# AndrewRLawrence/dp_gp_lvm

Hardware: AMD Instinct MI355X
Metric: ELBO evals/sec (N=2000,D=512,M=128,Q=10) (higher is better)
Workload: dtype f32 (psi-statistics: f16 hi/lo-split MFMA operands, fp32 accumulate) + f64 (Cholesky chain)

## Files before the change

### dp_gp_lvm_amd/csrc/psi2_pairs.hip

```cpp
#include <type_traits>
#include "internal.h"
#include "psi2_consts.h"
#include "psi2_chain_task.h"

typedef _Float16 pp_h8 __attribute__((ext_vector_type(8)));
typedef _Float16 pp_h2 __attribute__((ext_vector_type(2)));
typedef float pp_f16v __attribute__((ext_vector_type(16)));

#define PP_APAD 8
#define PP_LDS_HDR 512

#ifndef PP_G
#define PP_G(KS) ((KS) <= 4 ? 6 : ((KS) <= 6 ? 4 : 2))
#endif
#ifndef PP_WAVES
#define PP_WAVES 2
#endif
template <int KS> struct PairsCfg { static constexpr int G = PP_G(KS); };

#ifndef PP_NW8_MIN_TILES
#define PP_NW8_MIN_TILES 512
#endif
#ifndef PP_DEEP_PREFETCH
#define PP_DEEP_PREFETCH 1
#endif
#ifndef PP_SCALAR_ADD
#define PP_SCALAR_ADD 1
#endif

template <int KS, int GG, int NW>
__device__ __forceinline__ void pairs_load(pp_h8 (&bop)[GG][KS], int tb, const _Float16 *__restrict__ img, int l5, int half) {
#pragma unroll
    for (int g = 0; g < GG; ++g) {
        const pp_h8 *row = reinterpret_cast<const pp_h8 *>(img) + (size_t)(tb + NW * g) * KS * 64 + 32 * half + l5;
#pragma unroll
        for (int ks = 0; ks < KS; ++ks) bop[g][ks] = row[ks * 64];
    }
}

template <int KS, int GG, int NW>
__device__ __forceinline__ void pairs_group(int tb, pp_h8 (&bop)[GG][KS], int tb_next, const _Float16 *__restrict__ aimg,
                                            const _Float16 *__restrict__ img,
                                            const unsigned *__restrict__ pmap, const float *__restrict__ scale, int ntile,
                                            int l5, int half, float poison, float *__restrict__ out, int Mp, int chunk) {
    constexpr int SLP = 16 * KS, LDA = SLP + PP_APAD;
    static_assert(GG == 1 || (GG & 1) == 0, "ping-pong needs an even number of resident tiles");
    unsigned pm[GG];
    float sc[GG], old[GG];
#pragma unroll
    for (int g = 0; g < GG; ++g) {
        pm[g] = pmap[32 * (tb + NW * g) + l5];
        sc[g] = scale[32 * (tb + NW * g) + l5];
    }
#pragma unroll
    for (int g = 0; g < GG; ++g) {
        old[g] = 0.0f;
        if (chunk && pm[g] != 0xffffffffu && half == 0) old[g] = out[(size_t)(pm[g] >> 16) * Mp + (pm[g] & 0xffffu)];
    }
    float acc[GG][4];
#pragma unroll
    for (int g = 0; g < GG; ++g)
#pragma unroll
        for (int i = 0; i < 4; ++i) acc[g][i] = 0.0f;
    const _Float16 *arow = aimg + (size_t)l5 * LDA + 8 * half;
    auto load_a = [&](pp_h8 (&a)[KS], int nt) __attribute__((always_inline)) {
#ifdef PP_DIAG_NO_ALOAD
        if (nt > 1) return;
#endif
#pragma unroll
        for (int ks = 0; ks < KS; ++ks) a[ks] = *reinterpret_cast<const pp_h8 *>(arow + (size_t)nt * 32 * LDA + 16 * ks);
    };
    auto mma = [&](pp_f16v &c, const pp_h8 (&a)[KS], const pp_h8 (&bq)[KS]) __attribute__((always_inline)) {
#pragma unroll
        for (int v = 0; v < 16; ++v) c[v] = 0.0f;
#pragma unroll
        for (int ks = 0; ks < KS; ++ks) c = __builtin_amdgcn_mfma_f32_32x32x16_f16(a[ks], bq[ks], c, 0, 0, 0);
    };
    auto stage = [&](pp_f16v &cn, const pp_h8 (&a)[KS], const pp_h8 (&bq)[KS], float (&ac)[4], const pp_f16v &cu)
                     __attribute__((always_inline)) {
#pragma unroll
        for (int v = 0; v < 16; ++v) cn[v] = 0.0f;
#ifndef PP_MFMA_PER_STEP
#define PP_MFMA_PER_STEP 1
#endif
#pragma unroll
        for (int ks = 0; ks < KS; ks += PP_MFMA_PER_STEP) {
#ifndef PP_DIAG_NO_MFMA
#pragma unroll
            for (int k2 = ks; k2 < ks + PP_MFMA_PER_STEP && k2 < KS; ++k2)
                cn = __builtin_amdgcn_mfma_f32_32x32x16_f16(a[k2], bq[k2], cn, 0, 0, 0);
#endif
            __builtin_amdgcn_sched_barrier(0);
            const int kend = (ks + PP_MFMA_PER_STEP < KS) ? ks + PP_MFMA_PER_STEP : KS;
            const int v0 = (16 * ks) / KS, v1 = (16 * kend) / KS;
#pragma unroll
            for (int v = v0; v < v1; ++v) {
#ifdef PP_DIAG_NO_EXP
                const float e = cu[v];
#else
                const float e = __builtin_amdgcn_exp2f(cu[v]);
#endif
#if PP_SCALAR_ADD
                asm("v_add_f32 %0, %0, %1" : "+v"(ac[v & 3]) : "v"(e));
#else
                ac[v & 3] += e;
#endif
            }
            __builtin_amdgcn_sched_barrier(0);
        }
    };
    pp_f16v c0, c1;
    if constexpr (GG == 2 && PP_DEEP_PREFETCH) {
        pp_h8 a0[KS], a1[KS], a2[KS];
        load_a(a0, 0);
        load_a(a1, min(1, ntile - 1));
        mma(c0, a0, bop[0]);
#pragma unroll 1
        for (int nt = 0; nt < ntile; nt += 3) {
            load_a(a2, min(nt + 2, ntile - 1));
            stage(c1, a0, bop[1], acc[0], c0);
            stage(c0, a1, bop[0], acc[1], c1);
            if (nt + 1 >= ntile) break;
            load_a(a0, min(nt + 3, ntile - 1));
            stage(c1, a1, bop[1], acc[0], c0);
            stage(c0, a2, bop[0], acc[1], c1);
            if (nt + 2 >= ntile) break;
            load_a(a1, min(nt + 4, ntile - 1));
            stage(c1, a2, bop[1], acc[0], c0);
            stage(c0, a0, bop[0], acc[1], c1);
        }
    } else {
        pp_h8 a_0[KS], a_1[KS];
        load_a(a_0, 0);
        mma(c0, a_0, bop[0]);
        auto row = [&](const pp_h8 (&a_cur)[KS], const pp_h8 (&a_nxt)[KS]) __attribute__((always_inline)) {
            if constexpr (GG == 1) {
                stage(c1, a_nxt, bop[0], acc[0], c0);
                c0 = c1;
            } else {
#pragma unroll
                for (int g = 0; g < GG; g += 2) {
                    stage(c1, a_cur, bop[g + 1], acc[g], c0);
                    if (g + 2 < GG) stage(c0, a_cur, bop[g + 2], acc[g + 1], c1);
                    else stage(c0, a_nxt, bop[0], acc[g + 1], c1);
                }
            }
        };
#pragma unroll 1
        for (int nt = 0; nt < ntile; nt += 2) {
            load_a(a_1, min(nt + 1, ntile - 1));
            row(a_0, a_1);
            if (nt + 1 >= ntile) break;
            load_a(a_0, min(nt + 2, ntile - 1));
            row(a_1, a_0);
        }
    }
    if (tb_next >= 0) pairs_load<KS, GG, NW>(bop, tb_next, img, l5, half);
#pragma unroll
    for (int g = 0; g < GG; ++g) {
        float tot = (acc[g][0] + acc[g][1]) + (acc[g][2] + acc[g][3]);
        tot += __shfl_xor(tot, 32, 64);
        if (pm[g] != 0xffffffffu && half == 0)
            out[(size_t)(pm[g] >> 16) * Mp + (pm[g] & 0xffffu)] = old[g] + (sc[g] * tot + poison);
    }
}

template <typename TIN>
__global__ __launch_bounds__(256) void psi2_pair_scale_kernel(int M, int Q, const TIN *__restrict__ z,
                                                              const TIN *__restrict__ gamma, const TIN *__restrict__ alpha,
                                                              float *__restrict__ scale) {
    psi2_pair_scale_block<TIN, TIN>((int)blockIdx.y, (int)blockIdx.x, M, Q, z, gamma, alpha, scale);
}

template <typename TIN, int KS, int NW>
__global__ __launch_bounds__(64 * NW, PP_WAVES) void psi2_pairs_kernel(int N, int M, int Q, int B, const unsigned char *__restrict__ consts,
                                                            const TIN *__restrict__ mu, const TIN *__restrict__ s,
                                                            const TIN *__restrict__ gamma, const float *__restrict__ scale,
                                                            float *__restrict__ part, int Mp, int n_per_split, int n_splits,
                                                            int n_ranges, int tiles_per_range, int R, ChainKTask task) {
    constexpr int G = PairsCfg<KS>::G, SLP = 16 * KS, LDA = SLP + PP_APAD;
    extern __shared__ __align__(16) unsigned char smem_raw[];
    int item;
    if (psi2_task_1d(blockIdx.x, task.ws ? B : 0, task.last != 0, item)) {
#ifndef PP_NO_CHAIN
        if constexpr (std::is_same<TIN, double>::value && NW == 4) chain_k_task<2>(task, item, smem_raw);
#endif
        return;
    }
    const int b = item % B, sp = (item / B) % n_splits, rg = item / (B * n_splits);
    float *gq = reinterpret_cast<float *>(smem_raw);
    float *zc = gq + 32;
    _Float16 *aimg = reinterpret_cast<_Float16 *>(smem_raw + PP_LDS_HDR);
    const Psi2Consts C = psi2_consts_layout(M, Q);
    const _Float16 *img = reinterpret_cast<const _Float16 *>(consts + C.off_pairs);
    const unsigned *pmap = reinterpret_cast<const unsigned *>(consts + C.off_pmap);
    const float *sc_b = scale + (size_t)b * C.Ppad;
    const int t = threadIdx.x, lane = t & 63, l5 = lane & 31, half = lane >> 5;
    const int wv = __builtin_amdgcn_readfirstlane(t >> 6);
    if (t < 32) {
        gq[t] = (t < Q) ? (float)gamma[(size_t)b * Q + t] : 0.0f;
        zc[t] = reinterpret_cast<const float *>(consts)[t];
    }
    const int tiles_total = C.Ppad / 32;
    const int t0 = rg * tiles_per_range, t1 = min(tiles_total, t0 + tiles_per_range);
    const int nbeg = sp * n_per_split, nend = min(N, nbeg + n_per_split);
    float poison = 0.0f;
    float *out = part + ((size_t)sp * B + b) * (size_t)Mp * Mp;
    bool oor = false;
    __syncthreads();

    for (int n0 = nbeg, chunk = 0; n0 < nend; n0 += R, ++chunk) {
        const int rows = min(R, nend - n0), ntile = (rows + 31) >> 5;
        if (chunk) __syncthreads();
        for (int r = t; r < 32 * ntile; r += 64 * NW) {
            const int n = n0 + r;
            unsigned *dst = reinterpret_cast<unsigned *>(aimg + (size_t)r * LDA);
            float cc = -60000.0f;
            if (n < nend) {
                cc = 0.0f;
                for (int q = 0; q < Q; ++q) {
                    const float g = gq[q], sv = (float)s[(size_t)n * Q + q], mc = (float)mu[(size_t)n * Q + q] - zc[q];
                    const float den = 2.0f * g * sv + 1.0f, w = g / den;
                    const float a = dpgp_pin((float)(-0.25 * DPGP_LOG2E / PSI2_PAIR_S2_SCALE) * w);
                    const float bb = dpgp_pin((float)DPGP_LOG2E * w * mc);
                    cc -= bb * mc + 0.5f * __builtin_amdgcn_logf(den);
                    const _Float16 ah = (_Float16)a, alo = (_Float16)(a - (float)ah);
                    const _Float16 bh = (_Float16)bb, blo = (_Float16)(bb - (float)bh);
                    const pp_h2 w0 = {ah, ah}, w1 = {alo, bh}, w2 = {bh, blo};
                    dst[3 * q] = __builtin_bit_cast(unsigned, w0);
                    dst[3 * q + 1] = __builtin_bit_cast(unsigned, w1);
                    dst[3 * q + 2] = __builtin_bit_cast(unsigned, w2);
                }
                oor |= !(cc >= -8192.0f);
                cc = fmaxf(cc, -60000.0f);
            } else {
                for (int q = 0; q < 3 * Q; ++q) dst[q] = 0u;
            }
            cc = dpgp_pin(cc);
            const _Float16 ch = (_Float16)cc;
            const float r1 = dpgp_pin(cc - (float)ch);
            const _Float16 cm = (_Float16)r1;
            const pp_h2 cw = {ch, cm}, cw2 = {(_Float16)(r1 - (float)cm), (_Float16)0.0f};
            dst[3 * Q] = __builtin_bit_cast(unsigned, cw);
            for (int k = 3 * Q + 1; k < SLP / 2; ++k) dst[k] = 0u;
            if (6 * Q + 2 < SLP) dst[3 * Q + 1] = __builtin_bit_cast(unsigned, cw2);
        }
        if (__syncthreads_or(oor ? 1 : 0)) poison = __builtin_nanf("");

        int tb = t0 + wv;
        if (tb + NW * (G - 1) < t1) {
            pp_h8 bop[G][KS];
            pairs_load<KS, G, NW>(bop, tb, img, l5, half);
            for (; tb + NW * (G - 1) < t1; tb += NW * G) {
                const int nx = tb + NW * G;
                pairs_group<KS, G, NW>(tb, bop, nx + NW * (G - 1) < t1 ? nx : -1, aimg, img, pmap, sc_b, ntile, l5, half, poison, out,
                                   Mp, chunk);
            }
        }
        if constexpr (G > 2)
            for (; tb + NW < t1; tb += 2 * NW) {
                pp_h8 bop[2][KS];
                pairs_load<KS, 2, NW>(bop, tb, img, l5, half);
                pairs_group<KS, 2, NW>(tb, bop, -1, aimg, img, pmap, sc_b, ntile, l5, half, poison, out, Mp, chunk);
            }
        for (; tb < t1; tb += NW) {
            pp_h8 bop[1][KS];
            pairs_load<KS, 1, NW>(bop, tb, img, l5, half);
            pairs_group<KS, 1, NW>(tb, bop, -1, aimg, img, pmap, sc_b, ntile, l5, half, poison, out, Mp, chunk);
        }
    }
}

struct PairsGeom {
    int KS, R, n_ranges, tiles_per_range, NW;
    size_t lds;
};
static PairsGeom pairs_geom(int B, int N, int M, int Q, int ns, size_t chain_lds) {
    const Psi2Consts C = psi2_consts_layout(M, Q);
    PairsGeom g;
    g.KS = C.KS;
    const size_t row = sizeof(_Float16) * (size_t)(16 * C.KS + PP_APAD);
    size_t budget = 80 * 1024;
    if (const char *e = getenv("DPGP_PP_LDS_KB")) budget = (size_t)atoi(e) * 1024;
    if (chain_lds > budget) budget = chain_lds;
    int rmax = (int)((budget - PP_LDS_HDR) / row) & ~31;
    const int nper = dpgp_ceil_div(N, ns);
    g.NW = (!chain_lds && nper > rmax && C.Ppad / 32 >= PP_NW8_MIN_TILES) ? 8 : 4;
    if (const char *e = getenv("DPGP_PP_NW")) {
        const int v = atoi(e);
        if ((v == 4 || v == 8) && !(v == 8 && chain_lds)) g.NW = v;
    }
    if (g.NW == 8) {
        budget = 160 * 1024;
        rmax = (int)((budget - PP_LDS_HDR) / row) & ~31;
    }
    int r = dpgp_round_up(nper, 32);
    if (r > rmax) {
        const int chunks = dpgp_ceil_div(nper, rmax);
        r = dpgp_round_up(dpgp_ceil_div(nper, chunks), 32);
    }
    g.R = r;
    g.lds = PP_LDS_HDR + row * (size_t)r;
    if (chain_lds > g.lds) g.lds = chain_lds;
    const int tiles = C.Ppad / 32;
    int nr = chain_lds ? (B < 128 ? 512 - B : 512) / (B * ns) : dpgp_ceil_div(g.NW == 8 ? 256 : 512, B * ns);
    if (nr > dpgp_ceil_div(tiles, 32)) nr = dpgp_ceil_div(tiles, 32);
    if (nr < 1) nr = 1;
    if (const char *e = getenv("DPGP_PP_RANGES")) {
        const int v = atoi(e);
        if (v >= 1 && v <= tiles) nr = v;
    }
    g.tiles_per_range = dpgp_ceil_div(tiles, nr);
    g.n_ranges = dpgp_ceil_div(tiles, g.tiles_per_range);
    return g;
}

template <typename TIN, int KS, int NW>
static int launch_pairs_ks(int B, int N, int M, int Q, const TIN *mu, const TIN *s, const TIN *gamma, const float *scale,
                           float *part, int ns, const ChainKTask &task, const unsigned char *consts, const PairsGeom &g,
                           hipStream_t st) {
    const int Mp = dpgp_round_up(M, 16);
    const int nper = dpgp_ceil_div(N, ns);
    const long long nwg = (long long)B * ns * g.n_ranges + (task.ws ? B : 0);
    if (nwg > 0x7fffffffLL) return -1;
    auto kern = psi2_pairs_kernel<TIN, KS, NW>;
    if (NW == 8 && task.ws) return -16;
    if (g.lds > 48 * 1024 &&
        hipFuncSetAttribute(reinterpret_cast<const void *>(kern), hipFuncAttributeMaxDynamicSharedMemorySize, (int)g.lds) !=
            hipSuccess)
        return DPGP_ERR_LAUNCH;
    DPGP_PRELAUNCH(); hipLaunchKernelGGL(kern, dim3((unsigned)nwg), dim3(64 * NW), g.lds, st, N, M, Q, B, consts, mu, s, gamma, scale, part,
                       Mp, nper, ns, g.n_ranges, g.tiles_per_range, g.R, task);
    DPGP_LAUNCH_CHECK();
    return DPGP_OK;
}

size_t psi2_pairs_scale_bytes(int B, int M) {
    const size_t ppad = ((size_t)M * (M + 1) / 2 + 31) & ~(size_t)31;
    return dpgp_align256(sizeof(float) * (size_t)B * ppad);
}
template <typename TIN>
int launch_psi2_pairs(int B, int N, int M, int Q, const TIN *z, const TIN *mu, const TIN *s, const TIN *gamma,
                      const TIN *alpha, float *part, int ns, const ChainKTask &task, const unsigned char *consts, float *scale,
                      int scale_ready, hipStream_t st) {
    if (!consts || !scale) return -18;
    if (!scale_ready) {
        const Psi2Consts C = psi2_consts_layout(M, Q);
        DPGP_PRELAUNCH(); hipLaunchKernelGGL((psi2_pair_scale_kernel<TIN>), dim3(dpgp_ceil_div(C.Ppad, 256), B), dim3(256), 0, st, M, Q, z,
                           gamma, alpha, scale);
        DPGP_LAUNCH_CHECK();
    }
    size_t chain_lds = 0;
    if (task.ws) {
        if (!chain_k_resident(task.Mp, task.elem)) return -16;
        chain_lds = chain_k_lds_bytes(task.Mp, task.elem);
    }
    const PairsGeom g = pairs_geom(B, N, M, Q, ns, chain_lds);
    switch (g.KS) {
#define CASE(k)                                                                                                       \
    case k:                                                                                                           \
        return g.NW == 8 ? launch_pairs_ks<TIN, k, 8>(B, N, M, Q, mu, s, gamma, scale, part, ns, task, consts, g, st) \
                         : launch_pairs_ks<TIN, k, 4>(B, N, M, Q, mu, s, gamma, scale, part, ns, task, consts, g, st);
        CASE(2) CASE(4) CASE(6) CASE(8)
#undef CASE
    }
    return -4;
}
template int launch_psi2_pairs<float>(int, int, int, int, const float *, const float *, const float *, const float *,
                                      const float *, float *, int, const ChainKTask &, const unsigned char *, float *, int,
                                      hipStream_t);
template int launch_psi2_pairs<double>(int, int, int, int, const double *, const double *, const double *, const double *,
                                       const double *, float *, int, const ChainKTask &, const unsigned char *, float *, int,
                                       hipStream_t);
```

Before: 778.5.

## Stage mu/s rows through LDS with coalesced loads and defer old-output reads

Before building the A image, mu and s for the chunk are loaded cooperatively with coalesced, unrolled global reads and written into the tail of each LDS row. The per-row encode loop then reads them from LDS instead of making strided per-thread global loads. In the pair groups, the read of the previous partial output is moved after the MFMA loop, and explicit waitcnt calls let the MFMA loop wait only on the B-operand loads rather than on every outstanding memory op. This reuses LDS row padding as scratch and depends on hand-coded waitcnt encodings, which risks ordering bugs if the load counts assumed in those encodings are off.

New measurement: 785.5, median of 6. No clear change (+0.9%).

```diff
diff --git a/dp_gp_lvm_amd/csrc/psi2_pairs.hip b/dp_gp_lvm_amd/csrc/psi2_pairs.hip
--- a/dp_gp_lvm_amd/csrc/psi2_pairs.hip
+++ b/dp_gp_lvm_amd/csrc/psi2_pairs.hip
@@ -26,6 +26,10 @@
 #endif
 #ifndef PP_SCALAR_ADD
 #define PP_SCALAR_ADD 1
+#endif
+
+#ifndef PP_STAGE_U
+#define PP_STAGE_U 8
 #endif
 
 template <int KS, int GG, int NW>
@@ -46,16 +50,11 @@
     constexpr int SLP = 16 * KS, LDA = SLP + PP_APAD;
     static_assert(GG == 1 || (GG & 1) == 0, "ping-pong needs an even number of resident tiles");
     unsigned pm[GG];
-    float sc[GG], old[GG];
+    float sc[GG];
 #pragma unroll
     for (int g = 0; g < GG; ++g) {
         pm[g] = pmap[32 * (tb + NW * g) + l5];
         sc[g] = scale[32 * (tb + NW * g) + l5];
-    }
-#pragma unroll
-    for (int g = 0; g < GG; ++g) {
-        old[g] = 0.0f;
-        if (chunk && pm[g] != 0xffffffffu && half == 0) old[g] = out[(size_t)(pm[g] >> 16) * Mp + (pm[g] & 0xffffu)];
     }
     float acc[GG][4];
 #pragma unroll
@@ -109,12 +108,14 @@
             __builtin_amdgcn_sched_barrier(0);
         }
     };
+    auto bop_wait = [&]() __attribute__((always_inline)) { __builtin_amdgcn_s_waitcnt(0x0f70 | (2 * GG)); };
     pp_f16v c0, c1;
     if constexpr (GG == 2 && PP_DEEP_PREFETCH) {
         pp_h8 a0[KS], a1[KS], a2[KS];
         load_a(a0, 0);
         load_a(a1, min(1, ntile - 1));
         mma(c0, a0, bop[0]);
+        bop_wait();
 #pragma unroll 1
         for (int nt = 0; nt < ntile; nt += 3) {
             load_a(a2, min(nt + 2, ntile - 1));
@@ -133,6 +134,7 @@
         pp_h8 a_0[KS], a_1[KS];
         load_a(a_0, 0);
         mma(c0, a_0, bop[0]);
+        bop_wait();
         auto row = [&](const pp_h8 (&a_cur)[KS], const pp_h8 (&a_nxt)[KS]) __attribute__((always_inline)) {
             if constexpr (GG == 1) {
                 stage(c1, a_nxt, bop[0], acc[0], c0);
@@ -155,14 +157,25 @@
             row(a_1, a_0);
         }
     }
+    unsigned off[GG];
+    float old[GG];
+#pragma unroll
+    for (int g = 0; g < GG; ++g) {
+        off[g] = (pm[g] != 0xffffffffu && half == 0) ? (pm[g] >> 16) * (unsigned)Mp + (pm[g] & 0xffffu) : 0xffffffffu;
+        old[g] = 0.0f;
+        if (chunk && off[g] != 0xffffffffu) old[g] = out[off[g]];
+    }
     if (tb_next >= 0) pairs_load<KS, GG, NW>(bop, tb_next, img, l5, half);
+    float tot[GG];
 #pragma unroll
     for (int g = 0; g < GG; ++g) {
-        float tot = (acc[g][0] + acc[g][1]) + (acc[g][2] + acc[g][3]);
-        tot += __shfl_xor(tot, 32, 64);
-        if (pm[g] != 0xffffffffu && half == 0)
-            out[(size_t)(pm[g] >> 16) * Mp + (pm[g] & 0xffffu)] = old[g] + (sc[g] * tot + poison);
-    }
+        tot[g] = (acc[g][0] + acc[g][1]) + (acc[g][2] + acc[g][3]);
+        tot[g] += __shfl_xor(tot[g], 32, 64);
+    }
+    __builtin_amdgcn_s_waitcnt(0x0f70);
+#pragma unroll
+    for (int g = 0; g < GG; ++g)
+        if (off[g] != 0xffffffffu) out[off[g]] = old[g] + (sc[g] * tot[g] + poison);
 }
 
 template <typename TIN>
@@ -212,14 +225,48 @@
     for (int n0 = nbeg, chunk = 0; n0 < nend; n0 += R, ++chunk) {
         const int rows = min(R, nend - n0), ntile = (rows + 31) >> 5;
         if (chunk) __syncthreads();
+        const int SW = LDA / 2 - 2 * Q;
+        {
+            const int ne = rows * Q;
+            const TIN *mu0 = mu + (size_t)n0 * Q, *s0 = s + (size_t)n0 * Q;
+            int tq = t;
+            asm volatile("" : "+v"(tq));
+            const int er_d = __builtin_amdgcn_readfirstlane((64 * NW) / Q), eq_d = 64 * NW - er_d * Q;
+            int er = tq / Q, eq = tq - er * Q;
+            for (int e0 = t; e0 < ne; e0 += PP_STAGE_U * 64 * NW) {
+                TIN mv[PP_STAGE_U], sv[PP_STAGE_U];
+#pragma unroll
+                for (int u = 0; u < PP_STAGE_U; ++u) {
+                    const int e = min(e0 + u * 64 * NW, ne - 1);
+                    mv[u] = mu0[e];
+                    sv[u] = s0[e];
+                }
+#pragma unroll
+                for (int u = 0; u < PP_STAGE_U; ++u) {
+                    if (e0 + u * 64 * NW < ne) {
+                        float2 *slot = reinterpret_cast<float2 *>(reinterpret_cast<float *>(aimg + (size_t)er * LDA) + SW) + eq;
+                        *slot = make_float2((float)mv[u], (float)sv[u]);
+                    }
+                    er += er_d;
+                    eq += eq_d;
+                    if (eq >= Q) {
+                        eq -= Q;
+                        ++er;
+                    }
+                }
+            }
+        }
+        __syncthreads();
         for (int r = t; r < 32 * ntile; r += 64 * NW) {
             const int n = n0 + r;
             unsigned *dst = reinterpret_cast<unsigned *>(aimg + (size_t)r * LDA);
+            const float2 *in = reinterpret_cast<const float2 *>(reinterpret_cast<const float *>(dst) + SW);
             float cc = -60000.0f;
             if (n < nend) {
                 cc = 0.0f;
                 for (int q = 0; q < Q; ++q) {
-                    const float g = gq[q], sv = (float)s[(size_t)n * Q + q], mc = (float)mu[(size_t)n * Q + q] - zc[q];
+                    const float2 ms = in[q];
+                    const float g = gq[q], sv = ms.y, mc = ms.x - zc[q];
                     const float den = 2.0f * g * sv + 1.0f, w = g / den;
                     const float a = dpgp_pin((float)(-0.25 * DPGP_LOG2E / PSI2_PAIR_S2_SCALE) * w);
                     const float bb = dpgp_pin((float)DPGP_LOG2E * w * mc);
```
